# Florescence/UNet-Medical-Image-Contour-Segmentation-cpp

Measured on AMD Instinct MI355X. Metric: images/sec, 512x512 UNet fp32 inference (u8 tile -> u8 label map), higher is better.
Workload: dtype fp32; 1 GPU; BASELINE.json configs[1]: batch 16 x 512x512x1 u8 per GPU, 4-level UNet base 64, fp32, argmax label maps; global_batch=16, parallelism=dp1

## Files before the change

unet-medical-image-contour-segmentation-cpp_amd/csrc/conv_wino4s.hip:

```cpp
#include <cstdlib>
#include <type_traits>

#include "kernel_common.h"
#include "routing.h"
#include "wino4_common.h"

namespace miunet {

struct W4S {
    static constexpr int HEAD_ROW = 64 + 4;
    static constexpr size_t LDS_BYTES = sizeof(float) * (W4::VBUF + W4::RAW_FLOATS);
    static constexpr size_t LDS_BYTES_HEAD = sizeof(float) * (256 * HEAD_ROW + 4 * 64);
    static constexpr int FIRST_WIN = 20;
    static constexpr int FIRST_WMAX = WINO4S_FIRST_WMAX;
    static constexpr size_t LDS_BYTES_FIRST = LDS_BYTES + sizeof(float) * (FIRST_WIN * FIRST_WIN + 10 * FIRST_WMAX);
    static_assert(LDS_BYTES <= sizeof(float) * 256 * HEAD_ROW, "the head launch's allocation must cover the K loop's V + raw images");
};

template <bool HEAD, int UD, int EXP = 0, bool LATE = true, bool FIRST = false>
__global__ __launch_bounds__(256, 2) void conv3x3_wino4s_f32(const ConvArgs a, const int tiles_x, const int tiles_y,
                                                             const int m_tiles, const int nwg)
{
    constexpr int VROW = W4::VROW, VPOS = W4::VPOS;
    constexpr int HEAD_ROW = W4S::HEAD_ROW;
    static_assert(36 % UD == 0, "ring depth must divide the position count");
    extern __shared__ __attribute__((aligned(16))) float lds[];
    float *const Vs = lds;
    float *const Raw = lds + W4::VBUF;
    float *const Win = Raw + W4::RAW_FLOATS;
    float *const Wf = Win + W4S::FIRST_WIN * W4S::FIRST_WIN;

    const int tid = threadIdx.x;
    const int lane = tid & 63;
    const int wave = __builtin_amdgcn_readfirstlane(tid >> 6);
    const int j16 = lane & 15, kq = lane >> 4;

    int L = xcd_remap(blockIdx.x, nwg);
    const int n_tile = L / m_tiles;
    int m = L - n_tile * m_tiles;
    const int tx = m % tiles_x; m /= tiles_x;
    const int ty = m % tiles_y;
    const int b = m / tiles_y;
    const int bx0 = tx * 16, by0 = ty * 16;
    const int ncol0 = n_tile * 64 + 16 * wave + j16;
    const unsigned u_voff = (unsigned)(ncol0 * WINO4_KC + 4 * kq) * 4;
    const __amdgpu_buffer_rsrc_t in_rsrc = __builtin_amdgcn_make_buffer_rsrc(
        const_cast<float *>(a.in + (size_t)b * a.H * a.W * a.ldc), 0, a.H * a.W * a.ldc * 4, 0x00020000);

    unsigned raw_voff[W4::RAW_ITERS];
#pragma unroll
    for (int s = 0; s < W4::RAW_ITERS; ++s) {
        const int g = (wave + 4 * s) * 16 + (lane >> 2);
        const int py = g / W4::RAW_ROW, sl = g - py * W4::RAW_ROW;
        const int px = 4 * (sl % 5) + sl / 5;
        const int gy = by0 - 1 + py, gx = bx0 - 1 + px;
        const bool inb = g < W4::RAW_SLOTS && px < 18 && gy >= 0 && gy < a.H && gx >= 0 && gx < a.W;
        raw_voff[s] = inb ? (unsigned)(((gy * a.W + gx) * a.ldc + 4 * (lane & 3)) * 4) : 0xFFFFFFFFu;
    }
    auto first_patch = [&](int chunk) {
        const int cq = chunk * WINO4_KC + 4 * (lane & 3);
        const float *wq = Wf + cq;
#pragma unroll 1
        for (int s = 0; s < W4::RAW_ITERS; ++s) {
            if (wave + 4 * s >= W4::RAW_LOADS) break;
            const int g = (wave + 4 * s) * 16 + (lane >> 2);
            const int py = g / W4::RAW_ROW, sl = g - py * W4::RAW_ROW;
            const int px = 4 * (sl % 5) + sl / 5;
            const int gy = by0 - 1 + py, gx = bx0 - 1 + px;
            const bool inb = g < W4::RAW_SLOTS && px < 18 && gy >= 0 && gy < a.H && gx >= 0 && gx < a.W;
            f32x4 r = f32x4{ 0.f, 0.f, 0.f, 0.f };
            if (inb) {
                f32x4 acc = f32x4{ 0.f, 0.f, 0.f, 0.f };
                const float *wp = Win + py * W4S::FIRST_WIN + px;
#pragma unroll
                for (int t = 0; t < 9; ++t) acc += wp[(t / 3) * W4S::FIRST_WIN + t % 3] * *reinterpret_cast<const f32x4 *>(wq + t * a.Cin);
                const f32x4 a4 = acc + *reinterpret_cast<const f32x4 *>(wq + 9 * a.Cin);
                r.x = a4.x > 0.f ? a4.x : 0.f; r.y = a4.y > 0.f ? a4.y : 0.f; r.z = a4.z > 0.f ? a4.z : 0.f; r.w = a4.w > 0.f ? a4.w : 0.f;
            }
            *reinterpret_cast<f32x4 *>(Raw + (size_t)g * WINO4_KC + 4 * (lane & 3)) = r;
        }
    };
    typedef __attribute__((address_space(3))) void *lds_ptr;
    auto raw_dma_one = [&](int chunk, int s) {
        const int c0 = chunk * WINO4_KC;
        const bool c_ok = c0 + 4 * (lane & 3) < a.Cin;
        if (wave + 4 * s < W4::RAW_LOADS)
            __builtin_amdgcn_raw_ptr_buffer_load_lds(in_rsrc, (lds_ptr)(Raw + (wave + 4 * s) * 16 * WINO4_KC), 16,
                                                     c_ok ? raw_voff[s] : 0xFFFFFFFFu, c0 * 4, 0, 0);
    };

    const bool two = wave < 2;
    const int t_tile = lane >> 2, t_quad = lane & 3;
    const int row0 = two ? 1 : wave - 2, rstep = two ? 1 : 2;
    const float *const p_rd = Raw + (((4 * (t_tile >> 2) + row0) * W4::RAW_ROW + (t_tile & 3)) * 4 + t_quad) * 4;
    const int p_rstride = rstep * W4::RAW_ROW * WINO4_KC;
    const int xi_a = two ? (wave == 0 ? 1 : 3) : (wave == 2 ? 0 : 5);
    const float c_alpha = wave == 0 ? -4.f : -1.f, c_beta = wave == 0 ? 1.f : 2.f;
    float *const v_wr_a = Vs + xi_a * 6 * VPOS + t_tile * VROW + 4 * (t_quad ^ v_swz(t_tile));
    auto column_pass = [&](const f32x4 *c, float *dst) {
        const f32x4 e0 = c[4] - 4.f * c[2], e1 = c[3] - 4.f * c[1], e2 = pk_sub(c[4], c[2]), e3 = pk_sub(c[3], c[1]);
        *reinterpret_cast<f32x4 *>(dst + 0 * VPOS) = 4.f * c[0] - 5.f * c[2] + c[4];
        *reinterpret_cast<f32x4 *>(dst + 1 * VPOS) = e0 + e1;
        *reinterpret_cast<f32x4 *>(dst + 2 * VPOS) = pk_sub(e0, e1);
        *reinterpret_cast<f32x4 *>(dst + 3 * VPOS) = e2 + 2.f * e3;
        *reinterpret_cast<f32x4 *>(dst + 4 * VPOS) = e2 - 2.f * e3;
        *reinterpret_cast<f32x4 *>(dst + 5 * VPOS) = 4.f * c[1] - 5.f * c[3] + c[5];
    };
    auto transform = [&]() {
        f32x4 cR[2][6];
#pragma unroll
        for (int k = 0; k < 6; ++k) {
            const float *src = p_rd + ((k & 3) * 5 + (k >> 2)) * WINO4_KC;
            f32x4 d[4];
            d[0] = *reinterpret_cast<const f32x4 *>(src);
            d[1] = *reinterpret_cast<const f32x4 *>(src + p_rstride);
            d[2] = *reinterpret_cast<const f32x4 *>(src + 2 * p_rstride);
            d[3] = *reinterpret_cast<const f32x4 *>(src + 3 * p_rstride);
            f32x4 ra, rb;
            if (two) {
                const f32x4 ta = d[3] + c_alpha * d[1];
                const f32x4 tb = d[2] + c_alpha * d[0];
                ra = ta + c_beta * tb;
                rb = ta - c_beta * tb;
            } else {
                ra = 4.f * d[0] - 5.f * d[1] + d[2];
                rb = ra;
            }
            cR[0][k] = ra;
            cR[1][k] = rb;
        }
#pragma unroll
        for (int row = 0; row < 2; ++row) {
            if (row == 1 && !two) break;
            column_pass(cR[row], v_wr_a + row * 6 * VPOS);
        }
    };

    const unsigned u_pos_bytes = (unsigned)a.CoutPad * WINO4_KC * 4;
    const int nchunks = (a.Cin + WINO4_KC - 1) / WINO4_KC;
    const __amdgpu_buffer_rsrc_t u_rsrc =
        __builtin_amdgcn_make_buffer_rsrc(const_cast<float *>(a.wpk4), 0, (int)(nchunks * 36 * u_pos_bytes), 0x00020000);
    auto u_load = [&](int chunk, int p) {
        return __builtin_bit_cast(f32x4, __builtin_amdgcn_raw_buffer_load_b128(u_rsrc, u_voff, (chunk * 36 + p) * u_pos_bytes, 0));
    };
    const float *const v_rd = Vs + j16 * VROW + 4 * (kq ^ v_swz(j16));

    if constexpr (FIRST) {
        const uint8_t *imgb = a.first_img + (size_t)b * a.H * a.W;
        for (int i = tid; i < W4S::FIRST_WIN * W4S::FIRST_WIN; i += 256) {
            const int y = i / W4S::FIRST_WIN, x = i - y * W4S::FIRST_WIN, gy = by0 - 2 + y, gx = bx0 - 2 + x;
            Win[i] = (gy >= 0 && gy < a.H && gx >= 0 && gx < a.W) ? a.first_lut[imgb[(size_t)gy * a.W + gx]] : 0.f;
        }
        for (int i = tid; i < 10 * a.Cin; i += 256) Wf[i] = i < 9 * a.Cin ? a.first_w[i] : a.first_shift[i - 9 * a.Cin];
    } else {
#pragma unroll
        for (int s = 0; s < W4::RAW_ITERS; ++s) raw_dma_one(0, s);
    }
    f32x4 u[UD];
#pragma unroll
    for (int p = 0; p < UD; ++p) u[p] = u_load(0, p);

    f32x4 acc[36];
#pragma unroll
    for (int p = 0; p < 36; ++p) {
        const float init = (p == 7 && ncol0 < a.Cout) ? a.bias[ncol0] : 0.f;
#pragma unroll
        for (int r = 0; r < 4; ++r) acc[p][r] = init;
    }

    int chunk = 0;
    do {
        constexpr int LEFT = LATE ? 0 : UD;
        if constexpr (FIRST) {
            if (chunk == 0) __syncthreads();
            first_patch(chunk);
        } else {
            __builtin_amdgcn_s_waitcnt(0x0F70 | (LEFT & 15) | ((LEFT >> 4) << 14));
        }
        __syncthreads();
        transform();
        __syncthreads();
        const bool more = chunk + 1 < nchunks;
        const int nxt = more ? chunk + 1 : chunk;
        f32x4 av = *reinterpret_cast<const f32x4 *>(v_rd);
#pragma unroll
        for (int p = 0; p < 36; ++p) {
            f32x4 avn = av;
            if (p + 1 < 36) avn = *reinterpret_cast<const f32x4 *>(v_rd + (p + 1) * VPOS);
            if (!FIRST && more && !(EXP & 2)) {
                if (!LATE && p % 4 == 0 && p / 4 < W4::RAW_ITERS) raw_dma_one(chunk + 1, p / 4);
                if (LATE && p >= 36 - W4::RAW_ITERS) raw_dma_one(chunk + 1, p - (36 - W4::RAW_ITERS));
            }
            __builtin_amdgcn_sched_barrier(0);
            const f32x4 bv = u[p % UD];
#pragma unroll
            for (int s = 0; s < 4; ++s) acc[p] = __builtin_amdgcn_mfma_f32_16x16x4f32(av[s], bv[s], acc[p], 0, 0, 0);
            const int pn = p + UD;
            if constexpr (!(EXP & 1)) u[p % UD] = u_load(pn < 36 ? chunk : nxt, pn % 36);
            av = avn;
            __builtin_amdgcn_sched_barrier(0);
        }
    } while (++chunk < nchunks);

    const float relu_lo = a.relu ? 0.f : -__builtin_inff();
    const int Hp = a.H >> 1, Wp = a.W >> 1;
    const bool do_pool = a.pool_out != nullptr;
    const unsigned pix_bytes = (unsigned)a.ldo * 4, row_bytes = (unsigned)a.W * pix_bytes;
    const unsigned ppix_bytes = (unsigned)a.pool_ld * 4, prow_bytes = (unsigned)Wp * ppix_bytes;
    const __amdgpu_buffer_rsrc_t out_rsrc = __builtin_amdgcn_make_buffer_rsrc(a.out + (size_t)b * a.H * a.W * a.ldo, 0,
                                                                              a.H * a.W * a.ldo * 4, 0x00020000);
    const __amdgpu_buffer_rsrc_t pool_rsrc = __builtin_amdgcn_make_buffer_rsrc(
        do_pool ? a.pool_out + (size_t)b * Hp * Wp * a.pool_ld : a.out, 0, do_pool ? Hp * Wp * a.pool_ld * 4 : 0, 0x00020000);
    const int oy = by0 + 4 * kq;
    if constexpr (HEAD) __syncthreads();
    auto epilogue = [&](auto interior_tag) {
        constexpr bool INTERIOR = decltype(interior_tag)::value;
        const int ncol = ncol0;
        const bool n_ok = ncol < a.Cout;
        const unsigned vbase = n_ok ? (unsigned)((oy * a.W + bx0) * a.ldo + a.co_off + ncol) * 4 : 0xFFFFFFFFu;
        const unsigned pbase = n_ok ? (unsigned)(((oy >> 1) * Wp + (bx0 >> 1)) * a.pool_ld + ncol) * 4 : 0xFFFFFFFFu;
        unsigned vcol[4][4], pcol[4][2];
        if constexpr (!INTERIOR) {
#pragma unroll
            for (int r = 0; r < 4; ++r) {
#pragma unroll
                for (int k = 0; k < 4; ++k) vcol[r][k] = bx0 + 4 * r + k < a.W ? vbase : 0xFFFFFFFFu;
                pcol[r][0] = bx0 + 4 * r + 1 < a.W ? pbase : 0xFFFFFFFFu;
                pcol[r][1] = bx0 + 4 * r + 3 < a.W ? pbase : 0xFFFFFFFFu;
            }
        }
#pragma unroll
        for (int h2 = 0; h2 < 2; ++h2) {
            auto half = [&](const f32x4 &v) { return h2 ? v.hi : v.lo; };
            f32x2 t[4][6];
#pragma unroll
            for (int nu = 0; nu < 6; ++nu) {
                const f32x2 m0 = half(acc[nu]), m1 = half(acc[6 + nu]), m2 = half(acc[12 + nu]),
                            m3 = half(acc[18 + nu]), m4 = half(acc[24 + nu]), m5 = half(acc[30 + nu]);
                const f32x2 s12 = m1 + m2, d12 = pk_sub2(m1, m2), s34 = m3 + m4, d34 = pk_sub2(m3, m4);
                t[0][nu] = m0 + s12 + s34;
                t[1][nu] = d12 + 2.f * d34;
                t[2][nu] = s12 + 4.f * s34;
                t[3][nu] = d12 + 8.f * d34 + m5;
            }
            f32x2 carry0, carry1;
#pragma unroll
            for (int i = 0; i < 4; ++i) {
                const f32x2 s12 = t[i][1] + t[i][2], d12 = pk_sub2(t[i][1], t[i][2]), s34 = t[i][3] + t[i][4], d34 = pk_sub2(t[i][3], t[i][4]);
                f32x2 y[4];
                y[0] = t[i][0] + s12 + s34;
                y[1] = d12 + 2.f * d34;
                y[2] = s12 + 4.f * s34;
                y[3] = d12 + 8.f * d34 + t[i][5];
                const bool row_ok = INTERIOR || oy + i < a.H;
#pragma unroll
                for (int k = 0; k < 4; ++k)
#pragma unroll
                    for (int rr = 0; rr < 2; ++rr) {
                        const int r = 2 * h2 + rr;
                        const float v = fmaxf(y[k][rr], relu_lo);
                        y[k][rr] = v;
                        if constexpr (HEAD) {
                            lds[((4 * kq + i) * 16 + 4 * r + k) * HEAD_ROW + (ncol & 63)] = v;
                            continue;
                        }
                        unsigned voff = vbase;
                        if constexpr (!INTERIOR) voff = row_ok ? vcol[r][k] : 0xFFFFFFFFu;
                        __builtin_amdgcn_raw_buffer_store_b32(__builtin_bit_cast(unsigned, v), out_rsrc, voff,
                                                              i * row_bytes + (4 * r + k) * pix_bytes, ST_AUX);
                    }
                if (!HEAD && do_pool) {
                    f32x2 hm0, hm1;
#pragma unroll
                    for (int rr = 0; rr < 2; ++rr) { hm0[rr] = fmaxf(y[0][rr], y[1][rr]); hm1[rr] = fmaxf(y[2][rr], y[3][rr]); }
                    if ((i & 1) == 0) { carry0 = hm0; carry1 = hm1; }
                    else {
#pragma unroll
                        for (int rr = 0; rr < 2; ++rr) {
                            const int r = 2 * h2 + rr;
                            const float p0 = fmaxf(hm0[rr], carry0[rr]), p1 = fmaxf(hm1[rr], carry1[rr]);
                            unsigned v0 = pbase, v1 = pbase;
                            if constexpr (!INTERIOR) { v0 = row_ok ? pcol[r][0] : 0xFFFFFFFFu; v1 = row_ok ? pcol[r][1] : 0xFFFFFFFFu; }
                            __builtin_amdgcn_raw_buffer_store_b32(__builtin_bit_cast(unsigned, p0), pool_rsrc, v0,
                                                                  (i >> 1) * prow_bytes + (2 * r) * ppix_bytes, ST_AUX);
                            __builtin_amdgcn_raw_buffer_store_b32(__builtin_bit_cast(unsigned, p1), pool_rsrc, v1,
                                                                  (i >> 1) * prow_bytes + (2 * r + 1) * ppix_bytes, ST_AUX);
                        }
                    }
                }
            }
        }
    };
    if (HEAD || (by0 + 16 <= a.H && bx0 + 16 <= a.W)) epilogue(std::true_type{});
    else epilogue(std::false_type{});
    if constexpr (HEAD) {
        float *const Wh = lds + 256 * HEAD_ROW;
        if (tid < a.head_classes * 64) Wh[tid] = (tid & 63) < a.Cout ? a.head_w[(tid >> 6) * a.Cout + (tid & 63)] : 0.f;
        __syncthreads();
        f32x4 d4[4];
#pragma unroll
        for (int k = 0; k < 4; ++k) d4[k] = f32x4{ 0.f, 0.f, 0.f, 0.f };
        const float *yrow = lds + tid * HEAD_ROW;
#pragma unroll
        for (int c4 = 0; c4 < 16; ++c4) {
            const f32x4 yv = *reinterpret_cast<const f32x4 *>(yrow + 4 * c4);
#pragma unroll
            for (int k = 0; k < 4; ++k)
                if (k < a.head_classes) d4[k] += yv * *reinterpret_cast<const f32x4 *>(Wh + 64 * k + 4 * c4);
        }
        float d[4];
#pragma unroll
        for (int k = 0; k < 4; ++k) d[k] = k < a.head_classes ? ((d4[k].x + d4[k].y) + (d4[k].z + d4[k].w)) + a.head_b[k] : 0.f;
        const int py = by0 + (tid >> 4), px = bx0 + (tid & 15);
        if (py < a.H && px < a.W) {
            const size_t hw = (size_t)a.H * a.W, pin = (size_t)py * a.W + px;
            float best = -3.402823466e+38f;
            int idx = 0;
#pragma unroll
            for (int k = 0; k < 4; ++k) {
                if (k < a.head_classes) {
                    if (a.head_logits != nullptr) a.head_logits[((size_t)b * a.head_classes + k) * hw + pin] = d[k];
                    if (d[k] > best) { best = d[k]; idx = k; }
                }
            }
            a.head_labels[(size_t)b * hw + pin] = (uint8_t)idx;
        }
    }
}

template <bool HEAD>
static hipError_t launch_wino4s_cfg(const ConvArgs &a, hipStream_t s)
{
    const int tiles_x = (a.W + 15) / 16, tiles_y = (a.H + 15) / 16;
    const int m_tiles = tiles_x * tiles_y * a.B;
    const int n_tiles = (a.Cout + 63) / 64;
    const int nwg = m_tiles * n_tiles;
    size_t lds_bytes = HEAD ? W4S::LDS_BYTES_HEAD : W4S::LDS_BYTES;
    const bool first = a.first_img != nullptr;
    if (first) {
        if (HEAD || !conv3x3_wino4s_can_fuse_first(a, 1)) return hipErrorInvalidValue;
        lds_bytes = W4S::LDS_BYTES_FIRST;
    }
#ifdef MIUNET_EXPERIMENTS
    static const bool one_wg = [] { const char *e = getenv("MIUNET_WINO4S_ONE_WG"); return e && e[0] == '1'; }();
    if (one_wg) lds_bytes = 96 * 1024;
    static const int exp = [] { const char *e = getenv("MIUNET_W4S_EXP"); return e ? atoi(e) : 0; }();
    static const int ud = [] { const char *e = getenv("MIUNET_W4S_UD"); return e ? atoi(e) : 6; }();
#endif
    auto launch = [&](auto kern) {
        if (hipError_t e = ensure_dynamic_lds(kern, lds_bytes); e != hipSuccess) return e;
        hipLaunchKernelGGL(kern, dim3(nwg), dim3(256), lds_bytes, s, a, tiles_x, tiles_y, m_tiles, nwg);
        return hipGetLastError();
    };
#ifdef MIUNET_EXPERIMENTS
    if (exp == 1) return launch(conv3x3_wino4s_f32<HEAD, 3, 1, false>);
    if (exp == 2) return launch(conv3x3_wino4s_f32<HEAD, 3, 2, false>);
    if (exp == 3) return launch(conv3x3_wino4s_f32<HEAD, 3, 3, false>);
    if (ud == 3) return launch(conv3x3_wino4s_f32<HEAD, 3, 0, false>);
    if (ud == 60) return launch(conv3x3_wino4s_f32<HEAD, 6, 0, false>);
#endif
    if constexpr (!HEAD) { if (first) return launch(conv3x3_wino4s_f32<false, 6, 0, true, true>); }
    return launch(conv3x3_wino4s_f32<HEAD, 6>);
}

hipError_t launch_conv3x3_wino4s(const ConvArgs &a, hipStream_t s)
{
    if (a.wpk4 == nullptr || a.Cin % 4 || (a.first_img == nullptr && a.ldc % 4) || a.CoutPad % NPAD) return hipErrorInvalidValue;
    if (a.head_w != nullptr) {
        if (a.Cout > 64 || a.head_classes < 1 || a.head_classes > 4 || a.pool_out != nullptr || a.head_labels == nullptr)
            return hipErrorInvalidValue;
        return launch_wino4s_cfg<true>(a, s);
    }
    return launch_wino4s_cfg<false>(a, s);
}

}
```

unet-medical-image-contour-segmentation-cpp_amd/csrc/wino4_common.h:

```cpp
#pragma once
#include "kernel_common.h"

namespace miunet {

typedef float f32x2 __attribute__((ext_vector_type(2)));
typedef unsigned u32x4 __attribute__((ext_vector_type(4)));
__device__ __forceinline__ f32x4 pk_sub(const f32x4 a, const f32x4 b)
{
    f32x2 lo, hi;
    asm("v_pk_add_f32 %0, %1, %2 neg_lo:[0,1] neg_hi:[0,1]" : "=v"(lo) : "v"(a.lo), "v"(b.lo));
    asm("v_pk_add_f32 %0, %1, %2 neg_lo:[0,1] neg_hi:[0,1]" : "=v"(hi) : "v"(a.hi), "v"(b.hi));
    return __builtin_shufflevector(lo, hi, 0, 1, 2, 3);
}

__device__ __forceinline__ f32x2 pk_sub2(const f32x2 a, const f32x2 b)
{
    f32x2 r;
    asm("v_pk_add_f32 %0, %1, %2 neg_lo:[0,1] neg_hi:[0,1]" : "=v"(r) : "v"(a), "v"(b));
    return r;
}


__device__ __forceinline__ int v_swz(int tile) { return 2 * ((tile >> 2) & 1); }

struct W4 {
    static constexpr int TMB = 16;
    static constexpr int VROW = WINO4_KC;
    static constexpr int VPOS = TMB * VROW;
    static constexpr int VBUF = 36 * VPOS;
    static constexpr int RAWPIX = 18 * 18;
    static constexpr int RAW_ROW = 20;
    static constexpr int RAW_SLOTS = 18 * RAW_ROW;
    static constexpr int RAW_LOADS = (RAW_SLOTS + 15) / 16;
    static constexpr int RAW_FLOATS = RAW_LOADS * 16 * WINO4_KC;
    static constexpr int RAW_ITERS = (RAW_LOADS + 3) / 4;
    static constexpr size_t LDS_BYTES = sizeof(float) * (2 * VBUF + 2 * RAW_FLOATS);
};

}
```

profiles/summarize_pmc.py:

```python
#!/usr/bin/env python3
import argparse
import collections
import csv
import hashlib
import glob
import json
import os
import re

ROOT = os.path.dirname(os.path.dirname(os.path.abspath(__file__)))
SIMDS = 256 * 4
CLOCK_HZ = 2.4e9
SHADER_ENGINES = 32


def kernel_source_sha():
    h = hashlib.sha256()
    pkg = os.path.join(ROOT, "unet-medical-image-contour-segmentation-cpp_amd", "csrc")
    for p in sorted(glob.glob(os.path.join(pkg, "*")) + glob.glob(os.path.join(pkg, "asm", "*"))):
        if os.path.isfile(p):
            h.update(os.path.basename(p).encode())
            h.update(open(p, "rb").read())
    return h.hexdigest()[:16]


def short(name):
    m = re.match(r"_ZN(\d+)([A-Za-z_]\w*)", name)
    if m:
        ns = m.group(2)[:int(m.group(1))]
        rest = m.group(2)[int(m.group(1)):] + name[m.end():]
        m2 = re.match(r"(\d+)", rest)
        if m2:
            n = int(m2.group(1))
            fn = rest[len(m2.group(1)):len(m2.group(1)) + n]
            return f"{ns}::{fn}<{rest[len(m2.group(1)) + n:][:40]}>"
    return name.split("(")[0].replace("void ", "").strip()


def agg(path, counters):
    val = collections.defaultdict(lambda: collections.defaultdict(list))
    dur = collections.defaultdict(dict)
    for r in csv.DictReader(open(path)):
        k = short(r["Kernel_Name"])
        if r["Counter_Name"] in counters:
            val[k][r["Counter_Name"]].append(float(r["Counter_Value"]))
        dur[k][r["Dispatch_Id"]] = int(r["End_Timestamp"]) - int(r["Start_Timestamp"])
    return val, dur


def with_families(d):
    for k in list(d):
        fam = k.split("<")[0]
        if fam != k:
            tgt = d[fam + "<*>"]
            if isinstance(d[k], dict):
                for c, v in d[k].items():
                    if isinstance(v, list):
                        tgt.setdefault(c, []).extend(v)
                    else:
                        tgt[c] = v
    return d


def main():
    ap = argparse.ArgumentParser()
    ap.add_argument("--fetch")
    ap.add_argument("--write")
    ap.add_argument("--sq")
    ap.add_argument("--out", required=True)
    ap.add_argument("--command", default="")
    ap.add_argument("--sha", default=None, help="source hash of the tree the passes ran on (default: this tree's)")
    a = ap.parse_args()
    out = collections.defaultdict(dict)
    mean = lambda v: sum(v) / len(v)
    if a.fetch and a.write:
        f, _ = agg(a.fetch, {"FETCH_SIZE"})
        w, _ = agg(a.write, {"WRITE_SIZE"})
        f, w = with_families(f), with_families(w)
        for k in f:
            if k not in w or not f[k]["FETCH_SIZE"] or not w[k]["WRITE_SIZE"]:
                continue
            fetch = 2.0 * 1024.0 * mean(f[k]["FETCH_SIZE"])
            write = 1024.0 * mean(w[k]["WRITE_SIZE"])
            out[k].update({"launches_sampled": len(f[k]["FETCH_SIZE"]), "fetch_bytes_per_launch": fetch,
                           "write_bytes_per_launch": write, "hbm_bytes_per_launch": fetch + write})
    if a.sq:
        names = {"SQ_VALU_MFMA_BUSY_CYCLES", "SQ_BUSY_CYCLES", "SQ_WAVE_CYCLES", "SQ_WAIT_ANY", "SQ_WAIT_INST_ANY",
                 "SQ_ACTIVE_INST_ANY", "SQ_INSTS_VALU_MFMA_MOPS_F32", "SQ_INSTS_VALU_MFMA_MOPS_BF16", "SQ_INSTS_VALU_MFMA_MOPS_F16",
                 "SQ_INSTS_MFMA", "SQ_VALU_MFMA_COEXEC_CYCLES"}
        s, dur = agg(a.sq, names)
        for k in list(dur):
            s[k]["__dur"] = list(dur[k].values())
        s = with_families(s)
        for k, c in s.items():
            if not c.get("SQ_VALU_MFMA_BUSY_CYCLES") or not c.get("__dur"):
                continue
            busy, d_ns = mean(c["SQ_VALU_MFMA_BUSY_CYCLES"]), mean(c["__dur"])
            rec = {"sq_launches_sampled": len(c["__dur"]), "avg_launch_ns_under_pmc": d_ns, "mfma_busy_cycles_per_launch": busy,
                   "mfma_busy": busy / (SIMDS * d_ns * 1e-9 * CLOCK_HZ)}
            if c.get("SQ_BUSY_CYCLES"):
                sq_cycles = mean(c["SQ_BUSY_CYCLES"]) / SHADER_ENGINES
                rec["clock_ghz_from_sq_busy"] = sq_cycles / d_ns
                rec["mfma_busy_at_measured_clock"] = busy / (SIMDS * sq_cycles)
            for n in sorted(names - {"SQ_VALU_MFMA_BUSY_CYCLES"}):
                if c.get(n):
                    rec[n.lower() + "_per_launch"] = mean(c[n])
            out[k].update(rec)
    doc = {"kernel_source_sha": a.sha or kernel_source_sha(), "command": a.command,
           "method": "rocprofv3 --pmc, one counter group per run, --kernel-trace only; FETCH_SIZE doubled (gfx950), "
                     "mfma_busy = SQ_VALU_MFMA_BUSY_CYCLES / (1024 SIMDs x duration x 2.4 GHz)",
           "kernels": out}
    json.dump(doc, open(a.out, "w"), indent=1)
    print(json.dumps({k: v for k, v in out.items() if "<*>" in k or "<" not in k}, indent=1))


if __name__ == "__main__":
    main()
```

Baseline: 1038 images/s.

## Rebalance Winograd input transform across waves and precompute first-layer patch indices

Rewrites the Winograd F(4,3) input transform so each wave handles a balanced mix of two-row and one-row work on f32x2 lanes, replacing the previous split where two waves did twice the work of the others. It also precomputes per-slot window offsets for the fused first-layer patch into an LDS decode table, so the bounds and index arithmetic is not redone on every chunk. The MFMA loop switches to a two-entry A-operand ring instead of a register copy. The cost is a larger LDS allocation for the fused-first launch, guarded by a static assert, and more, narrower LDS accesses.

```diff
diff --git a/unet-medical-image-contour-segmentation-cpp_amd/csrc/conv_wino4s.hip b/unet-medical-image-contour-segmentation-cpp_amd/csrc/conv_wino4s.hip
--- a/unet-medical-image-contour-segmentation-cpp_amd/csrc/conv_wino4s.hip
+++ b/unet-medical-image-contour-segmentation-cpp_amd/csrc/conv_wino4s.hip
@@ -13,7 +13,8 @@
     static constexpr size_t LDS_BYTES_HEAD = sizeof(float) * (256 * HEAD_ROW + 4 * 64);
     static constexpr int FIRST_WIN = 20;
     static constexpr int FIRST_WMAX = WINO4S_FIRST_WMAX;
-    static constexpr size_t LDS_BYTES_FIRST = LDS_BYTES + sizeof(float) * (FIRST_WIN * FIRST_WIN + 10 * FIRST_WMAX);
+    static constexpr size_t LDS_BYTES_FIRST = LDS_BYTES + sizeof(float) * (FIRST_WIN * FIRST_WIN + 10 * FIRST_WMAX + W4::RAW_ITERS * 256);
+    static_assert(2 * LDS_BYTES_FIRST <= 160 * 1024, "two workgroups of the fused-first launch share a compute unit's LDS");
     static_assert(LDS_BYTES <= sizeof(float) * 256 * HEAD_ROW, "the head launch's allocation must cover the K loop's V + raw images");
 };
 
@@ -29,6 +30,7 @@
     float *const Raw = lds + W4::VBUF;
     float *const Win = Raw + W4::RAW_FLOATS;
     float *const Wf = Win + W4S::FIRST_WIN * W4S::FIRST_WIN;
+    int *const Dec = reinterpret_cast<int *>(Wf + 10 * W4S::FIRST_WMAX);
 
     const int tid = threadIdx.x;
     const int lane = tid & 63;
@@ -64,20 +66,28 @@
         for (int s = 0; s < W4::RAW_ITERS; ++s) {
             if (wave + 4 * s >= W4::RAW_LOADS) break;
             const int g = (wave + 4 * s) * 16 + (lane >> 2);
+            const int win = Dec[s * 256 + tid];
+            f32x4 r = f32x4{ 0.f, 0.f, 0.f, 0.f };
+            if (win >= 0) {
+                f32x4 acc = f32x4{ 0.f, 0.f, 0.f, 0.f };
+                const float *wp = Win + win;
+#pragma unroll
+                for (int t = 0; t < 9; ++t) acc += wp[(t / 3) * W4S::FIRST_WIN + t % 3] * *reinterpret_cast<const f32x4 *>(wq + t * a.Cin);
+                const f32x4 a4 = acc + *reinterpret_cast<const f32x4 *>(wq + 9 * a.Cin);
+                r.x = a4.x > 0.f ? a4.x : 0.f; r.y = a4.y > 0.f ? a4.y : 0.f; r.z = a4.z > 0.f ? a4.z : 0.f; r.w = a4.w > 0.f ? a4.w : 0.f;
+            }
+            *reinterpret_cast<f32x4 *>(Raw + (size_t)g * WINO4_KC + 4 * (lane & 3)) = r;
+        }
+    };
+    auto first_decode = [&]() {
+#pragma unroll
+        for (int s = 0; s < W4::RAW_ITERS; ++s) {
+            const int g = (wave + 4 * s) * 16 + (lane >> 2);
             const int py = g / W4::RAW_ROW, sl = g - py * W4::RAW_ROW;
             const int px = 4 * (sl % 5) + sl / 5;
             const int gy = by0 - 1 + py, gx = bx0 - 1 + px;
             const bool inb = g < W4::RAW_SLOTS && px < 18 && gy >= 0 && gy < a.H && gx >= 0 && gx < a.W;
-            f32x4 r = f32x4{ 0.f, 0.f, 0.f, 0.f };
-            if (inb) {
-                f32x4 acc = f32x4{ 0.f, 0.f, 0.f, 0.f };
-                const float *wp = Win + py * W4S::FIRST_WIN + px;
-#pragma unroll
-                for (int t = 0; t < 9; ++t) acc += wp[(t / 3) * W4S::FIRST_WIN + t % 3] * *reinterpret_cast<const f32x4 *>(wq + t * a.Cin);
-                const f32x4 a4 = acc + *reinterpret_cast<const f32x4 *>(wq + 9 * a.Cin);
-                r.x = a4.x > 0.f ? a4.x : 0.f; r.y = a4.y > 0.f ? a4.y : 0.f; r.z = a4.z > 0.f ? a4.z : 0.f; r.w = a4.w > 0.f ? a4.w : 0.f;
-            }
-            *reinterpret_cast<f32x4 *>(Raw + (size_t)g * WINO4_KC + 4 * (lane & 3)) = r;
+            Dec[s * 256 + tid] = inb ? py * W4S::FIRST_WIN + px : -1;
         }
     };
     typedef __attribute__((address_space(3))) void *lds_ptr;
@@ -89,51 +99,51 @@
                                                      c_ok ? raw_voff[s] : 0xFFFFFFFFu, c0 * 4, 0, 0);
     };
 
-    const bool two = wave < 2;
-    const int t_tile = lane >> 2, t_quad = lane & 3;
-    const int row0 = two ? 1 : wave - 2, rstep = two ? 1 : 2;
-    const float *const p_rd = Raw + (((4 * (t_tile >> 2) + row0) * W4::RAW_ROW + (t_tile & 3)) * 4 + t_quad) * 4;
-    const int p_rstride = rstep * W4::RAW_ROW * WINO4_KC;
-    const int xi_a = two ? (wave == 0 ? 1 : 3) : (wave == 2 ? 0 : 5);
-    const float c_alpha = wave == 0 ? -4.f : -1.f, c_beta = wave == 0 ? 1.f : 2.f;
-    float *const v_wr_a = Vs + xi_a * 6 * VPOS + t_tile * VROW + 4 * (t_quad ^ v_swz(t_tile));
-    auto column_pass = [&](const f32x4 *c, float *dst) {
-        const f32x4 e0 = c[4] - 4.f * c[2], e1 = c[3] - 4.f * c[1], e2 = pk_sub(c[4], c[2]), e3 = pk_sub(c[3], c[1]);
-        *reinterpret_cast<f32x4 *>(dst + 0 * VPOS) = 4.f * c[0] - 5.f * c[2] + c[4];
-        *reinterpret_cast<f32x4 *>(dst + 1 * VPOS) = e0 + e1;
-        *reinterpret_cast<f32x4 *>(dst + 2 * VPOS) = pk_sub(e0, e1);
-        *reinterpret_cast<f32x4 *>(dst + 3 * VPOS) = e2 + 2.f * e3;
-        *reinterpret_cast<f32x4 *>(dst + 4 * VPOS) = e2 - 2.f * e3;
-        *reinterpret_cast<f32x4 *>(dst + 5 * VPOS) = 4.f * c[1] - 5.f * c[3] + c[5];
+    const int t_odd = wave & 1, t_g2 = wave >> 1;
+    const int t_lt = lane >> 3, t_h = lane & 7;
+    auto t_rd = [&](int tile, int row0) { return Raw + ((4 * (tile >> 2) + row0) * W4::RAW_ROW + (tile & 3)) * WINO4_KC + 2 * t_h; };
+    auto t_wr = [&](int tile, int xi) { return Vs + xi * 6 * VPOS + tile * VROW + 4 * ((t_h >> 1) ^ v_swz(tile)) + 2 * (t_h & 1); };
+    const float *const p_rd2 = t_rd(8 * t_g2 + t_lt, 1), *const p_rd1 = t_rd(8 * (1 - t_g2) + t_lt, t_odd);
+    float *const v_wr2 = t_wr(8 * t_g2 + t_lt, t_odd ? 3 : 1), *const v_wr1 = t_wr(8 * (1 - t_g2) + t_lt, t_odd ? 5 : 0);
+    const float c_alpha = t_odd ? -1.f : -4.f, c_beta = t_odd ? 2.f : 1.f;
+    constexpr int P_ROW = W4::RAW_ROW * WINO4_KC;
+    auto column_pass = [&](const auto *c, float *dst) {
+        using T = std::remove_cv_t<std::remove_reference_t<decltype(c[0])>>;
+        const T e0 = c[4] - 4.f * c[2], e1 = c[3] - 4.f * c[1], e2 = pk_sub(c[4], c[2]), e3 = pk_sub(c[3], c[1]);
+        *reinterpret_cast<T *>(dst + 0 * VPOS) = 4.f * c[0] - 5.f * c[2] + c[4];
+        *reinterpret_cast<T *>(dst + 1 * VPOS) = e0 + e1;
+        *reinterpret_cast<T *>(dst + 2 * VPOS) = pk_sub(e0, e1);
+        *reinterpret_cast<T *>(dst + 3 * VPOS) = e2 + 2.f * e3;
+        *reinterpret_cast<T *>(dst + 4 * VPOS) = e2 - 2.f * e3;
+        *reinterpret_cast<T *>(dst + 5 * VPOS) = 4.f * c[1] - 5.f * c[3] + c[5];
     };
     auto transform = [&]() {
-        f32x4 cR[2][6];
+        f32x2 cR[2][6], cS[6];
 #pragma unroll
         for (int k = 0; k < 6; ++k) {
-            const float *src = p_rd + ((k & 3) * 5 + (k >> 2)) * WINO4_KC;
-            f32x4 d[4];
-            d[0] = *reinterpret_cast<const f32x4 *>(src);
-            d[1] = *reinterpret_cast<const f32x4 *>(src + p_rstride);
-            d[2] = *reinterpret_cast<const f32x4 *>(src + 2 * p_rstride);
-            d[3] = *reinterpret_cast<const f32x4 *>(src + 3 * p_rstride);
-            f32x4 ra, rb;
-            if (two) {
-                const f32x4 ta = d[3] + c_alpha * d[1];
-                const f32x4 tb = d[2] + c_alpha * d[0];
-                ra = ta + c_beta * tb;
-                rb = ta - c_beta * tb;
-            } else {
-                ra = 4.f * d[0] - 5.f * d[1] + d[2];
-                rb = ra;
-            }
-            cR[0][k] = ra;
-            cR[1][k] = rb;
-        }
-#pragma unroll
-        for (int row = 0; row < 2; ++row) {
-            if (row == 1 && !two) break;
-            column_pass(cR[row], v_wr_a + row * 6 * VPOS);
-        }
+            const float *src = p_rd2 + ((k & 3) * 5 + (k >> 2)) * WINO4_KC;
+            f32x2 d[4];
+            d[0] = *reinterpret_cast<const f32x2 *>(src);
+            d[1] = *reinterpret_cast<const f32x2 *>(src + P_ROW);
+            d[2] = *reinterpret_cast<const f32x2 *>(src + 2 * P_ROW);
+            d[3] = *reinterpret_cast<const f32x2 *>(src + 3 * P_ROW);
+            const f32x2 ta = d[3] + c_alpha * d[1];
+            const f32x2 tb = d[2] + c_alpha * d[0];
+            cR[0][k] = ta + c_beta * tb;
+            cR[1][k] = ta - c_beta * tb;
+        }
+#pragma unroll
+        for (int k = 0; k < 6; ++k) {
+            const float *src = p_rd1 + ((k & 3) * 5 + (k >> 2)) * WINO4_KC;
+            f32x2 d[3];
+            d[0] = *reinterpret_cast<const f32x2 *>(src);
+            d[1] = *reinterpret_cast<const f32x2 *>(src + 2 * P_ROW);
+            d[2] = *reinterpret_cast<const f32x2 *>(src + 4 * P_ROW);
+            cS[k] = 4.f * d[0] - 5.f * d[1] + d[2];
+        }
+#pragma unroll
+        for (int row = 0; row < 2; ++row) column_pass(cR[row], v_wr2 + row * 6 * VPOS);
+        column_pass(cS, v_wr1);
     };
 
     const unsigned u_pos_bytes = (unsigned)a.CoutPad * WINO4_KC * 4;
@@ -152,6 +162,7 @@
             Win[i] = (gy >= 0 && gy < a.H && gx >= 0 && gx < a.W) ? a.first_lut[imgb[(size_t)gy * a.W + gx]] : 0.f;
         }
         for (int i = tid; i < 10 * a.Cin; i += 256) Wf[i] = i < 9 * a.Cin ? a.first_w[i] : a.first_shift[i - 9 * a.Cin];
+        first_decode();
     } else {
 #pragma unroll
         for (int s = 0; s < W4::RAW_ITERS; ++s) raw_dma_one(0, s);
@@ -182,11 +193,11 @@
         __syncthreads();
         const bool more = chunk + 1 < nchunks;
         const int nxt = more ? chunk + 1 : chunk;
-        f32x4 av = *reinterpret_cast<const f32x4 *>(v_rd);
+        f32x4 av[2];
+        av[0] = *reinterpret_cast<const f32x4 *>(v_rd);
 #pragma unroll
         for (int p = 0; p < 36; ++p) {
-            f32x4 avn = av;
-            if (p + 1 < 36) avn = *reinterpret_cast<const f32x4 *>(v_rd + (p + 1) * VPOS);
+            if (p + 1 < 36) av[(p + 1) & 1] = *reinterpret_cast<const f32x4 *>(v_rd + (p + 1) * VPOS);
             if (!FIRST && more && !(EXP & 2)) {
                 if (!LATE && p % 4 == 0 && p / 4 < W4::RAW_ITERS) raw_dma_one(chunk + 1, p / 4);
                 if (LATE && p >= 36 - W4::RAW_ITERS) raw_dma_one(chunk + 1, p - (36 - W4::RAW_ITERS));
@@ -194,10 +205,9 @@
             __builtin_amdgcn_sched_barrier(0);
             const f32x4 bv = u[p % UD];
 #pragma unroll
-            for (int s = 0; s < 4; ++s) acc[p] = __builtin_amdgcn_mfma_f32_16x16x4f32(av[s], bv[s], acc[p], 0, 0, 0);
+            for (int s = 0; s < 4; ++s) acc[p] = __builtin_amdgcn_mfma_f32_16x16x4f32(av[p & 1][s], bv[s], acc[p], 0, 0, 0);
             const int pn = p + UD;
             if constexpr (!(EXP & 1)) u[p % UD] = u_load(pn < 36 ? chunk : nxt, pn % 36);
-            av = avn;
             __builtin_amdgcn_sched_barrier(0);
         }
     } while (++chunk < nchunks);
diff --git a/unet-medical-image-contour-segmentation-cpp_amd/csrc/wino4_common.h b/unet-medical-image-contour-segmentation-cpp_amd/csrc/wino4_common.h
--- a/unet-medical-image-contour-segmentation-cpp_amd/csrc/wino4_common.h
+++ b/unet-medical-image-contour-segmentation-cpp_amd/csrc/wino4_common.h
@@ -19,6 +19,7 @@
     asm("v_pk_add_f32 %0, %1, %2 neg_lo:[0,1] neg_hi:[0,1]" : "=v"(r) : "v"(a), "v"(b));
     return r;
 }
+__device__ __forceinline__ f32x2 pk_sub(const f32x2 a, const f32x2 b) { return pk_sub2(a, b); }
 
 
 __device__ __forceinline__ int v_swz(int tile) { return 2 * ((tile >> 2) & 1); }
```

New measurement: 1042 images/s (median of 4 runs). Within noise of the previous version (+0.3%).

## Precompute first-layer patch geometry in LDS, peel bias init, specialize head class count

Applied to the files above, without the earlier changes.

The fused first-layer path now computes per-slot patch offsets once into an LDS geometry table, handles two slots per iteration with shared weight loads, and pads first-layer weights to a fixed stride so the inner loop uses compile-time offsets. The main MFMA loop peels chunk 0 so bias and zero initialisation are folded into the first MFMA instead of a separate accumulator-init pass. The head 1x1 dot product is specialised by class count through a switch, which removes runtime predicates. Together these cut integer and VALU overhead in the conv kernel, at the cost of more LDS for the first-layer launch (now asserted to fit two workgroups per CU) and larger code.

```diff
diff --git a/profiles/summarize_pmc.py b/profiles/summarize_pmc.py
--- a/profiles/summarize_pmc.py
+++ b/profiles/summarize_pmc.py
@@ -87,7 +87,7 @@
     if a.sq:
         names = {"SQ_VALU_MFMA_BUSY_CYCLES", "SQ_BUSY_CYCLES", "SQ_WAVE_CYCLES", "SQ_WAIT_ANY", "SQ_WAIT_INST_ANY",
                  "SQ_ACTIVE_INST_ANY", "SQ_INSTS_VALU_MFMA_MOPS_F32", "SQ_INSTS_VALU_MFMA_MOPS_BF16", "SQ_INSTS_VALU_MFMA_MOPS_F16",
-                 "SQ_INSTS_MFMA", "SQ_VALU_MFMA_COEXEC_CYCLES"}
+                 "SQ_INSTS_MFMA", "SQ_VALU_MFMA_COEXEC_CYCLES", "SQ_INSTS_VALU"}
         s, dur = agg(a.sq, names)
         for k in list(dur):
             s[k]["__dur"] = list(dur[k].values())
diff --git a/unet-medical-image-contour-segmentation-cpp_amd/csrc/conv_wino4s.hip b/unet-medical-image-contour-segmentation-cpp_amd/csrc/conv_wino4s.hip
--- a/unet-medical-image-contour-segmentation-cpp_amd/csrc/conv_wino4s.hip
+++ b/unet-medical-image-contour-segmentation-cpp_amd/csrc/conv_wino4s.hip
@@ -13,7 +13,9 @@
     static constexpr size_t LDS_BYTES_HEAD = sizeof(float) * (256 * HEAD_ROW + 4 * 64);
     static constexpr int FIRST_WIN = 20;
     static constexpr int FIRST_WMAX = WINO4S_FIRST_WMAX;
-    static constexpr size_t LDS_BYTES_FIRST = LDS_BYTES + sizeof(float) * (FIRST_WIN * FIRST_WIN + 10 * FIRST_WMAX);
+    static constexpr int FIRST_GEO = 6 * 256;
+    static constexpr size_t LDS_BYTES_FIRST = LDS_BYTES + sizeof(float) * (FIRST_WIN * FIRST_WIN + 10 * FIRST_WMAX + FIRST_GEO + 4);
+    static_assert(2 * LDS_BYTES_FIRST <= 160 * 1024, "two workgroups per compute unit");
     static_assert(LDS_BYTES <= sizeof(float) * 256 * HEAD_ROW, "the head launch's allocation must cover the K loop's V + raw images");
 };
 
@@ -29,6 +31,7 @@
     float *const Raw = lds + W4::VBUF;
     float *const Win = Raw + W4::RAW_FLOATS;
     float *const Wf = Win + W4S::FIRST_WIN * W4S::FIRST_WIN;
+    int *const Geo = reinterpret_cast<int *>(Wf + 10 * W4S::FIRST_WMAX);
 
     const int tid = threadIdx.x;
     const int lane = tid & 63;
@@ -48,36 +51,65 @@
         const_cast<float *>(a.in + (size_t)b * a.H * a.W * a.ldc), 0, a.H * a.W * a.ldc * 4, 0x00020000);
 
     unsigned raw_voff[W4::RAW_ITERS];
-#pragma unroll
-    for (int s = 0; s < W4::RAW_ITERS; ++s) {
-        const int g = (wave + 4 * s) * 16 + (lane >> 2);
-        const int py = g / W4::RAW_ROW, sl = g - py * W4::RAW_ROW;
-        const int px = 4 * (sl % 5) + sl / 5;
-        const int gy = by0 - 1 + py, gx = bx0 - 1 + px;
-        const bool inb = g < W4::RAW_SLOTS && px < 18 && gy >= 0 && gy < a.H && gx >= 0 && gx < a.W;
-        raw_voff[s] = inb ? (unsigned)(((gy * a.W + gx) * a.ldc + 4 * (lane & 3)) * 4) : 0xFFFFFFFFu;
-    }
-    auto first_patch = [&](int chunk) {
-        const int cq = chunk * WINO4_KC + 4 * (lane & 3);
-        const float *wq = Wf + cq;
-#pragma unroll 1
+    if constexpr (!FIRST) {
+#pragma unroll
         for (int s = 0; s < W4::RAW_ITERS; ++s) {
-            if (wave + 4 * s >= W4::RAW_LOADS) break;
             const int g = (wave + 4 * s) * 16 + (lane >> 2);
             const int py = g / W4::RAW_ROW, sl = g - py * W4::RAW_ROW;
             const int px = 4 * (sl % 5) + sl / 5;
             const int gy = by0 - 1 + py, gx = bx0 - 1 + px;
             const bool inb = g < W4::RAW_SLOTS && px < 18 && gy >= 0 && gy < a.H && gx >= 0 && gx < a.W;
-            f32x4 r = f32x4{ 0.f, 0.f, 0.f, 0.f };
-            if (inb) {
-                f32x4 acc = f32x4{ 0.f, 0.f, 0.f, 0.f };
-                const float *wp = Win + py * W4S::FIRST_WIN + px;
-#pragma unroll
-                for (int t = 0; t < 9; ++t) acc += wp[(t / 3) * W4S::FIRST_WIN + t % 3] * *reinterpret_cast<const f32x4 *>(wq + t * a.Cin);
-                const f32x4 a4 = acc + *reinterpret_cast<const f32x4 *>(wq + 9 * a.Cin);
-                r.x = a4.x > 0.f ? a4.x : 0.f; r.y = a4.y > 0.f ? a4.y : 0.f; r.z = a4.z > 0.f ? a4.z : 0.f; r.w = a4.w > 0.f ? a4.w : 0.f;
-            }
-            *reinterpret_cast<f32x4 *>(Raw + (size_t)g * WINO4_KC + 4 * (lane & 3)) = r;
+            raw_voff[s] = inb ? (unsigned)(((gy * a.W + gx) * a.ldc + 4 * (lane & 3)) * 4) : 0xFFFFFFFFu;
+        }
+    }
+    const unsigned lim_y = (unsigned)min(a.H, by0 + 17), lim_x = (unsigned)min(a.W, bx0 + 17);
+    auto slot_geom = [&](int s, int &py, int &px) {
+        const int G = (wave + 4 * s) * 16;
+        const int Q = G / W4::RAW_ROW;
+        const int x = G - Q * W4::RAW_ROW + (lane >> 2);
+        const bool wrap = x >= W4::RAW_ROW;
+        const int sl = wrap ? x - W4::RAW_ROW : x;
+        const int q5 = __mul24(sl, 13) >> 6;
+        px = 4 * sl - __mul24(q5, 19);
+        py = Q + (wrap ? 1 : 0);
+        return (unsigned)(by0 - 1 + py) < lim_y && (unsigned)(bx0 - 1 + px) < lim_x;
+    };
+    float *const piece_wr = Raw + (wave * 16 + (lane >> 2)) * WINO4_KC + 4 * (lane & 3);
+    constexpr int PIECE_STRIDE = 4 * 16 * WINO4_KC;
+    auto first_geometry = [&]() {
+#pragma unroll
+        for (int s = 0; s < W4::RAW_ITERS; ++s) {
+            if (wave + 4 * s >= W4::RAW_LOADS) break;
+            int py, px;
+            const bool inb = slot_geom(s, py, px);
+            Geo[s * 256 + tid] = inb ? py * W4S::FIRST_WIN + px : -1;
+            if (!inb) *reinterpret_cast<f32x4 *>(piece_wr + s * PIECE_STRIDE) = f32x4{ 0.f, 0.f, 0.f, 0.f };
+        }
+    };
+    auto first_patch = [&](int chunk) {
+        const float *wq = Wf + chunk * WINO4_KC + 4 * (lane & 3);
+        float *const dummy = reinterpret_cast<float *>(Geo + W4S::FIRST_GEO);
+        auto finish = [&](const f32x4 acc, const f32x4 shift, int g, float *dst) {
+            const f32x4 a4 = acc + shift;
+            f32x4 r;
+            r.x = a4.x > 0.f ? a4.x : 0.f; r.y = a4.y > 0.f ? a4.y : 0.f; r.z = a4.z > 0.f ? a4.z : 0.f; r.w = a4.w > 0.f ? a4.w : 0.f;
+            *reinterpret_cast<f32x4 *>(g >= 0 ? dst : dummy) = r;
+        };
+#pragma unroll 1
+        for (int s = 0; s < W4::RAW_ITERS; s += 2) {
+            const bool pair = wave + 4 * (s + 1) < W4::RAW_LOADS;
+            const int g0 = Geo[s * 256 + tid], g1 = pair ? Geo[(s + 1) * 256 + tid] : -1;
+            const float *wp0 = Win + max(g0, 0), *wp1 = Win + max(g1, 0);
+            f32x4 acc0 = f32x4{ 0.f, 0.f, 0.f, 0.f }, acc1 = acc0;
+#pragma unroll
+            for (int t = 0; t < 9; ++t) {
+                const f32x4 w4 = *reinterpret_cast<const f32x4 *>(wq + t * W4S::FIRST_WMAX);
+                acc0 += wp0[(t / 3) * W4S::FIRST_WIN + t % 3] * w4;
+                acc1 += wp1[(t / 3) * W4S::FIRST_WIN + t % 3] * w4;
+            }
+            const f32x4 shift = *reinterpret_cast<const f32x4 *>(wq + 9 * W4S::FIRST_WMAX);
+            finish(acc0, shift, g0, piece_wr + s * PIECE_STRIDE);
+            finish(acc1, shift, g1, piece_wr + (s + 1) * PIECE_STRIDE);
         }
     };
     typedef __attribute__((address_space(3))) void *lds_ptr;
@@ -151,7 +183,11 @@
             const int y = i / W4S::FIRST_WIN, x = i - y * W4S::FIRST_WIN, gy = by0 - 2 + y, gx = bx0 - 2 + x;
             Win[i] = (gy >= 0 && gy < a.H && gx >= 0 && gx < a.W) ? a.first_lut[imgb[(size_t)gy * a.W + gx]] : 0.f;
         }
-        for (int i = tid; i < 10 * a.Cin; i += 256) Wf[i] = i < 9 * a.Cin ? a.first_w[i] : a.first_shift[i - 9 * a.Cin];
+        for (int i = tid; i < 10 * W4S::FIRST_WMAX; i += 256) {
+            const int t = i / W4S::FIRST_WMAX, c = i % W4S::FIRST_WMAX;
+            if (c < a.Cin) Wf[i] = t < 9 ? a.first_w[t * a.Cin + c] : a.first_shift[c];
+        }
+        first_geometry();
     } else {
 #pragma unroll
         for (int s = 0; s < W4::RAW_ITERS; ++s) raw_dma_one(0, s);
@@ -160,15 +196,40 @@
 #pragma unroll
     for (int p = 0; p < UD; ++p) u[p] = u_load(0, p);
 
+    constexpr bool PEEL0 = !FIRST;
     f32x4 acc[36];
-#pragma unroll
-    for (int p = 0; p < 36; ++p) {
-        const float init = (p == 7 && ncol0 < a.Cout) ? a.bias[ncol0] : 0.f;
-#pragma unroll
-        for (int r = 0; r < 4; ++r) acc[p][r] = init;
+    const float bias_v = ncol0 < a.Cout ? a.bias[ncol0] : 0.f;
+    const f32x4 acc0 = f32x4{ 0.f, 0.f, 0.f, 0.f }, acc_bias = f32x4{ bias_v, bias_v, bias_v, bias_v };
+    if constexpr (!PEEL0) {
+#pragma unroll
+        for (int p = 0; p < 36; ++p) acc[p] = p == 7 ? acc_bias : acc0;
     }
 
     int chunk = 0;
+    bool more;
+    int nxt;
+    auto mfma_phase = [&](auto peel_tag) {
+        constexpr bool PEEL = decltype(peel_tag)::value;
+        f32x4 av = *reinterpret_cast<const f32x4 *>(v_rd);
+#pragma unroll
+        for (int p = 0; p < 36; ++p) {
+            f32x4 avn = av;
+            if (p + 1 < 36) avn = *reinterpret_cast<const f32x4 *>(v_rd + (p + 1) * VPOS);
+            if (!FIRST && more && !(EXP & 2)) {
+                if (!LATE && p % 4 == 0 && p / 4 < W4::RAW_ITERS) raw_dma_one(chunk + 1, p / 4);
+                if (LATE && p >= 36 - W4::RAW_ITERS) raw_dma_one(chunk + 1, p - (36 - W4::RAW_ITERS));
+            }
+            __builtin_amdgcn_sched_barrier(0);
+            const f32x4 bv = u[p % UD];
+#pragma unroll
+            for (int s = 0; s < 4; ++s)
+                acc[p] = __builtin_amdgcn_mfma_f32_16x16x4f32(av[s], bv[s], PEEL && s == 0 ? (p == 7 ? acc_bias : acc0) : acc[p], 0, 0, 0);
+            const int pn = p + UD;
+            if constexpr (!(EXP & 1)) u[p % UD] = u_load(pn < 36 ? chunk : nxt, pn % 36);
+            av = avn;
+            __builtin_amdgcn_sched_barrier(0);
+        }
+    };
     do {
         constexpr int LEFT = LATE ? 0 : UD;
         if constexpr (FIRST) {
@@ -180,26 +241,10 @@
         __syncthreads();
         transform();
         __syncthreads();
-        const bool more = chunk + 1 < nchunks;
-        const int nxt = more ? chunk + 1 : chunk;
-        f32x4 av = *reinterpret_cast<const f32x4 *>(v_rd);
-#pragma unroll
-        for (int p = 0; p < 36; ++p) {
-            f32x4 avn = av;
-            if (p + 1 < 36) avn = *reinterpret_cast<const f32x4 *>(v_rd + (p + 1) * VPOS);
-            if (!FIRST && more && !(EXP & 2)) {
-                if (!LATE && p % 4 == 0 && p / 4 < W4::RAW_ITERS) raw_dma_one(chunk + 1, p / 4);
-                if (LATE && p >= 36 - W4::RAW_ITERS) raw_dma_one(chunk + 1, p - (36 - W4::RAW_ITERS));
-            }
-            __builtin_amdgcn_sched_barrier(0);
-            const f32x4 bv = u[p % UD];
-#pragma unroll
-            for (int s = 0; s < 4; ++s) acc[p] = __builtin_amdgcn_mfma_f32_16x16x4f32(av[s], bv[s], acc[p], 0, 0, 0);
-            const int pn = p + UD;
-            if constexpr (!(EXP & 1)) u[p % UD] = u_load(pn < 36 ? chunk : nxt, pn % 36);
-            av = avn;
-            __builtin_amdgcn_sched_barrier(0);
-        }
+        more = chunk + 1 < nchunks;
+        nxt = more ? chunk + 1 : chunk;
+        if (PEEL0 && chunk == 0) mfma_phase(std::true_type{});
+        else mfma_phase(std::false_type{});
     } while (++chunk < nchunks);
 
     const float relu_lo = a.relu ? 0.f : -__builtin_inff();
@@ -297,20 +342,28 @@
         float *const Wh = lds + 256 * HEAD_ROW;
         if (tid < a.head_classes * 64) Wh[tid] = (tid & 63) < a.Cout ? a.head_w[(tid >> 6) * a.Cout + (tid & 63)] : 0.f;
         __syncthreads();
-        f32x4 d4[4];
-#pragma unroll
-        for (int k = 0; k < 4; ++k) d4[k] = f32x4{ 0.f, 0.f, 0.f, 0.f };
         const float *yrow = lds + tid * HEAD_ROW;
-#pragma unroll
-        for (int c4 = 0; c4 < 16; ++c4) {
-            const f32x4 yv = *reinterpret_cast<const f32x4 *>(yrow + 4 * c4);
-#pragma unroll
-            for (int k = 0; k < 4; ++k)
-                if (k < a.head_classes) d4[k] += yv * *reinterpret_cast<const f32x4 *>(Wh + 64 * k + 4 * c4);
-        }
-        float d[4];
-#pragma unroll
-        for (int k = 0; k < 4; ++k) d[k] = k < a.head_classes ? ((d4[k].x + d4[k].y) + (d4[k].z + d4[k].w)) + a.head_b[k] : 0.f;
+        float d[4] = { 0.f, 0.f, 0.f, 0.f };
+        auto head_dot = [&](auto classes_tag) {
+            constexpr int NK = decltype(classes_tag)::value;
+            f32x4 d4[NK];
+#pragma unroll
+            for (int k = 0; k < NK; ++k) d4[k] = f32x4{ 0.f, 0.f, 0.f, 0.f };
+#pragma unroll
+            for (int c4 = 0; c4 < 16; ++c4) {
+                const f32x4 yv = *reinterpret_cast<const f32x4 *>(yrow + 4 * c4);
+#pragma unroll
+                for (int k = 0; k < NK; ++k) d4[k] += yv * *reinterpret_cast<const f32x4 *>(Wh + 64 * k + 4 * c4);
+            }
+#pragma unroll
+            for (int k = 0; k < NK; ++k) d[k] = ((d4[k].x + d4[k].y) + (d4[k].z + d4[k].w)) + a.head_b[k];
+        };
+        switch (a.head_classes) {
+        case 1: head_dot(std::integral_constant<int, 1>{}); break;
+        case 2: head_dot(std::integral_constant<int, 2>{}); break;
+        case 3: head_dot(std::integral_constant<int, 3>{}); break;
+        default: head_dot(std::integral_constant<int, 4>{}); break;
+        }
         const int py = by0 + (tid >> 4), px = bx0 + (tid & 15);
         if (py < a.H && px < a.W) {
             const size_t hw = (size_t)a.H * a.W, pin = (size_t)py * a.W + px;
```

Result: no change. 1035 images/s before, 1043 images/s after, median of 6 (+0.7%).
